# yeyupiaoling/VoiceprintRecognition-PaddlePaddle

Hardware: NVIDIA H100
Metric: utterances/sec ECAPA-TDNN Fbank80 3s embed extract (higher is better)
Workload: dtype bf16x3 (split-bf16 operands, fp32 accumulate; fp32-grade)

## Files before the change

voiceprintrecognition-paddlepaddle_b200/csrc/common.h:

```cpp
#pragma once
#include <cuda.h>
#include <cuda_bf16.h>
#include <cuda_runtime.h>
#include <stdint.h>
#include <stdlib.h>

#include <algorithm>
#include <string>
#include <utility>

#include "../../include/ppv_b200.h"

namespace ppv {

void set_error(const std::string& msg);
int fail(int code, const std::string& msg);

#define PPV_CUDA_OK(expr)                                                                             \
    do {                                                                                              \
        cudaError_t _e = (expr);                                                                      \
        if (_e != cudaSuccess)                                                                        \
            return ::ppv::fail(PPV_ECUDA, std::string(#expr) + ": " + cudaGetErrorString(_e));        \
    } while (0)
#define PPV_LAUNCH_OK(what)                                                                           \
// ... 134 lines not shown
    for (int bn = max_bn; bn > 64; bn /= 2)
        if (N % bn == 0) return bn;
    return 64;
}

int encode_planes_map(CUtensorMap* m, const Planes& t, int box_rows);
int encode_planes_map_ex(CUtensorMap* m, const Planes& t, int box_cols, int box_rows, int swizzle_bytes);

struct Res2Params {
    CUtensorMap mapA[2];
    CUtensorMap mapW;
    int a_col[2];
    int nsrc, dil;
    int l2_prefetch;
    int M, m_tiles;
    Epilogue epi;
};
int res2conv_build(Res2Params* rp, const GemmSource* srcs, int nsrc, const Planes& W, int M, int dil, const Epilogue& epi);
int res2conv_launch(const Res2Params& rp, int precision, int num_sms, cudaStream_t st);

struct Conv3x3Params {
    CUtensorMap mapX;
    CUtensorMap mapW;
    int x_col0;
    int B, H, W, Hp, Wp;
    int nph, npw, patches;
    Epilogue epi;
};
bool conv3x3_c32_supported(int Cin, int Cout, int H, int W);
int conv3x3_build(Conv3x3Params* cp, const Planes& x, int x_col0, const Planes& Wt, int B, int H, int W, int Hp, int Wp, const Epilogue& epi);
int conv3x3_launch(const Conv3x3Params& cp, int precision, int num_sms, cudaStream_t st);

constexpr int RES2CHAIN_MAX = 7;
struct Res2ChainParams {
    CUtensorMap mapX;
    CUtensorMap mapXt, mapY, mapYtail;
    CUtensorMap mapW[RES2CHAIN_MAX];
    const float* bias[RES2CHAIN_MAX];
    const float* bn_scale[RES2CHAIN_MAX];
    const float* bn_shift[RES2CHAIN_MAX];
    Planes x;
    Planes y;
    int nconv, width, B, T, P, Tp, dil, ntiles;
    int paired;
    unsigned long long* trace;
};
int res2chain_build(Res2ChainParams* cp, const Planes& x, const Planes& y, const Planes* W, const float* const* bias, const float* const* bn_scale,
                    const float* const* bn_shift, int nconv, int B, int T, int P, int Tp, int dil, bool paired);
int res2chain_launch(const Res2ChainParams& cp, int precision, int num_sms, cudaStream_t st);
bool res2chain_fits(int T, int P);
bool res2chain_pair_fits(int T, int P);
void res2chain_trace_dump(const Res2ChainParams& cp);

int pointwise_launch(const GemmSource* srcs, int nsrc, const Planes& W, int64_t M, int N, const Epilogue& ep, int num_sms, cudaStream_t st);
struct PwStep {
    GemmSource srcs[2];
    int nsrc = 0, N = 0;
    int64_t M = 0;
    Planes W;
    Epilogue ep;
};
inline int pointwise_launch(const PwStep& s, int num_sms, cudaStream_t st) { return pointwise_launch(s.srcs, s.nsrc, s.W, s.M, s.N, s.ep, num_sms, st); }
bool pointwise_step_build(PwStep* s, const GemmSource* srcs, int nsrc, const Planes& W, int N, int64_t M, const Epilogue& ep);

bool skinny_linear_supported(int M, int N, int K, const Epilogue& ep);
int skinny_linear_launch(const Planes& x, int x_col0, const Planes& W, int M, int N, int K, const Epilogue& ep, cudaStream_t st);

struct AspFusedParams {
    CUtensorMap mapW;
    CUtensorMap mapAtt;
    CUtensorMap mapX;
    Planes x;
    Planes gstat;
    const float* bn_scale;
    const float* bn_shift;
    Planes out;
    float* out_raw;
    int B, T, P, Tp, C, K;
    float eps;
    const int* nvalid;
};

int asp_fused_build(AspFusedParams* p, const Planes& W, const Planes& att, const Planes& x, const Planes& gstat, const float* bn_scale,
                    const float* bn_shift, const Planes& out, float* out_raw, int B, int T, int P, int Tp, int C, int K, float eps);
int asp_fused_launch(const AspFusedParams& p, int precision, int num_sms, cudaStream_t st);

int launch_pack_features(const float* feat, int B, int T, int F, const Planes& out, int P, int Tp, cudaStream_t st);
int launch_colstats(const Planes& x, int col0, int C, int B, int T, int P, int Tp, int mode, float eps, float* out_f32,
                    const Planes& out_pl, cudaStream_t st, float inv_count = 0.f, const int* nvalid = nullptr);
int launch_lengths_to_counts(const float* lengths, int B, int T, int* nvalid, cudaStream_t st);
int launch_se_scale_res(const Planes& z, const float* scale, const Planes& res, int rc0, const Planes& out, int oc0, int C,
                        int Tp, int64_t rows, int num_sms, cudaStream_t st, int relu = 0, float relu_max = 0.f);
int launch_asp_pool(const float* logits, int64_t lg_ld, const Planes& x, int C, int B, int T, int P, int Tp, float eps,
                    const float* bn_scale, const float* bn_shift, const Planes& out_pl, float* out_raw, cudaStream_t st);
int launch_planes_to_f32(const Planes& x, int col0, int C, int B, int T, int P, int Tp, float* out, cudaStream_t st);
int launch_f32_to_planes(const float* src, int64_t rows, int cols, const Planes& out, cudaStream_t st);

struct Fbank;
int fbank_create(const ppv_fbank_cfg* cfg, Fbank** out);
void fbank_destroy(Fbank* h);
int fbank_num_frames(const Fbank* h, int L);
int fbank_n_mels(const Fbank* h);
int fbank_run(Fbank* h, const float* wav, const float* lens_ratio, int B, int L, float* raw, float* out_f32,
              const Planes& out_pl, int P, int Tp, cudaStream_t st, const int* valid_frames = nullptr);

size_t audio_prep_workspace_bytes(int B, int max_new_len);
// ... 72 lines not shown
```

voiceprintrecognition-paddlepaddle_b200/csrc/ecapa.cu:

```cuda
#include <stdlib.h>
#include <string.h>

#include "common.h"
#include "model_common.h"

namespace ppv {

namespace {

struct ConvW : GemmWeights {
    float* bn_scale = nullptr;
    float* bn_shift = nullptr;
};

struct KSpec {
    int src;
    int col0, ncols, row_off;
    int w_cin0, w_cnt, w_tap;
};

enum Buf { B_FEAT, B_X0, B_H, B_Y, B_Z, B_CAT, B_MFA, B_ATT, B_GSTAT, B_POOL, B_SEM, B_SEH, B_COUNT };

struct Step {
    enum Kind { GEMM, SKINNY, RES2, RES2CHAIN, SE_SQUEEZE, SE_SCALE, ASP_GLOBAL, ASP_FUSED, POOL_STATS } kind;
    Planes sk_x, sk_w;
    int sk_col0 = 0, sk_M = 0, sk_N = 0, sk_K = 0;
    Epilogue sk_ep;
    GemmParams gp;
    AspFusedParams ap;
    Res2Params rp;
    Res2ChainParams cp;
    int blk = 0;
};

struct EcBuffers {
    Planes bufs[B_COUNT];
    float *se_mean = nullptr, *se_scale = nullptr, *fold_out = nullptr, *pooled_raw = nullptr, *raw_logmel = nullptr;
    int* nvalid = nullptr;
};

}

struct EcapaModel : Model {
    ppv_ecapa_cfg cfg;
    int C = 0, C3 = 0, width = 0, scale = 0, Fp = 0, P = 0, att = 0, se = 0;
    ConvW conv0, tdnn1[3], res2[3][8], tdnn2[3], se1[3], se2[3], mfa, fold, att1, att2, fc;
    float *aspbn_scale = nullptr, *aspbn_shift = nullptr;
    std::vector<Step> steps;
    EcBuffers buf;
    int Tp = 0;
    bool prof_on = false;
    std::vector<cudaEvent_t> prof_ev;
    std::vector<int> prof_kind;
    size_t prof_used = 0;
    int64_t launches_gemm = 0, launches_other = 0;

    explicit EcapaModel(const ppv_ecapa_cfg& c) : Model("ecapa", c.precision), cfg(c) {}
    ~EcapaModel() override {
        for (cudaEvent_t e : prof_ev) cudaEventDestroy(e);
    }
    int embd_dim() const override { return cfg.embd_dim; }
    size_t workspace_bytes(int B, int T) const override;
    int forward_ex(const float* feat, Fbank* fb, const float* wav, const float* lens_ratio, int B, int T, int L, float* emb, void* ws,
                   size_t ws_bytes, cudaStream_t st, const float* lengths);

  protected:
    bool prepare_weights(ArenaBuilder& ab) override;
    int build_plan(int B, int T, void* ws, size_t ws_bytes, cudaStream_t st) override;
    int run_steps(const float* feat, cudaStream_t st) override { return run(feat, nullptr, nullptr, nullptr, 0, nullptr, st); }
    int tap(const std::string& n, float* out, size_t out_elems, cudaStream_t st) override;
    int run(const float* feat, Fbank* fb, const float* wav, const float* lens_ratio, int L, const float* lengths, cudaStream_t st);
};

void ppv_ecapa_default_cfg_impl(ppv_ecapa_cfg* c) {
    c->input_size = 80;
    c->embd_dim = 192;
    const int ch[5] = {512, 512, 512, 512, 1536}, ks[5] = {5, 3, 3, 3, 1}, dl[5] = {1, 2, 3, 4, 1};
    for (int i = 0; i < 5; ++i) {
        c->channels[i] = ch[i];
        c->kernel_sizes[i] = ks[i];
        c->dilations[i] = dl[i];
    }
    c->attention_channels = 128;
    c->res2net_scale = 8;
// ... 175 lines not shown
    eb->bufs[B_H] = cv.planes(R, C);
    eb->bufs[B_Y] = cv.planes(R, C);
    eb->bufs[B_Z] = cv.planes(R, C);
    eb->bufs[B_CAT] = cv.planes(R, C3);
    eb->bufs[B_MFA] = cv.planes(R, C3);
    eb->bufs[B_ATT] = cv.planes(R, m->att);
    eb->bufs[B_GSTAT] = cv.planes(B, 2 * C3);
    eb->bufs[B_POOL] = cv.planes(B, 2 * C3);
    eb->bufs[B_SEM] = cv.planes(B, C);
    eb->bufs[B_SEH] = cv.planes(B, m->se);
    eb->se_mean = static_cast<float*>(cv.take(size_t(B) * C * 4));
    eb->se_scale = static_cast<float*>(cv.take(size_t(B) * C * 4));
    eb->fold_out = static_cast<float*>(cv.take(mc_align_up(B, 128) * m->att * 4));
    eb->pooled_raw = static_cast<float*>(cv.take(size_t(B) * 2 * C3 * 4));
    eb->raw_logmel = static_cast<float*>(cv.take(size_t(B) * T * m->cfg.input_size * 4));
    *emb_out = static_cast<float*>(cv.take(mc_align_up(B, 128) * m->cfg.embd_dim * 4));
    eb->nvalid = static_cast<int*>(cv.take(size_t(B) * sizeof(int)));
}

constexpr int ECAPA_MAX_BN = 128;

}

size_t EcapaModel::workspace_bytes(int B, int T) const {
    if (B <= 0 || T <= 0) return 0;
    WsCarver cv;
    EcBuffers eb;
    float* emb;
    carve(this, cv, B, T, &eb, &emb);
    return mc_align_up(cv.off, 256);
}

int EcapaModel::build_plan(int B, int T, void* ws, size_t ws_bytes, cudaStream_t st) {
    EcapaModel* const m = this;
    PPV_REQUIRE(T > m->P, "ecapa: too few frames for the reflect padding");
    const size_t need = workspace_bytes(B, T);
    PPV_REQUIRE(ws && ws_bytes >= need, "ecapa: workspace too small (see ppv_model_workspace_bytes)");
    PPV_REQUIRE((reinterpret_cast<uintptr_t>(ws) & 255) == 0, "ecapa: workspace must be 256-byte aligned");
    WsCarver cv;
    cv.base = static_cast<uint8_t*>(ws);
    carve(m, cv, B, T, &m->buf, &m->emb_out);
    m->Tp = T + 2 * m->P;
    PPV_CUDA_OK(cudaMemsetAsync(ws, 0, need, st));
    m->steps.clear();
    const int Tp = m->Tp, P = m->P, C = m->C, C3 = m->C3, w = m->width;
    const int64_t R = int64_t(B) * Tp;
    const char* r2env = getenv("PPV_RES2_GEMM");
    const bool use_res2_kernel = (w == 64) && !(r2env && r2env[0] == '1');
    const char* rcenv = getenv("PPV_RES2_CHAIN");
    const bool use_res2_chain = use_res2_kernel && m->scale == 8 && res2chain_fits(T, P) && !(rcenv && rcenv[0] == '0');
    const bool res2_paired = use_res2_chain && res2chain_pair_fits(T, P) && !(rcenv && strcmp(rcenv, "single") == 0);
    const char* skenv = getenv("PPV_SKINNY");
    const bool use_skinny = !(skenv && skenv[0] == '0');

    auto add_gemm = [&](const ConvW& cw, const std::vector<KSpec>& ks, const Planes* src_override, int override_col0, int M,
                        Epilogue ep) -> int {
        std::vector<GemmSource> srcs;
        for (const KSpec& s : ks) {
            GemmSource g;
            if (s.src < 0) {
                g.t = *src_override;
                g.col0 = override_col0 + s.col0;
            } else {
                g.t = m->buf.bufs[s.src];
                g.col0 = s.col0;
            }
            g.ncols = s.ncols;
            g.row_off = s.row_off;
            srcs.push_back(g);
        }
        ep.bias = cw.bias;
        if (ep.relu) {
            ep.bn_scale = cw.bn_scale;
            ep.bn_shift = cw.bn_shift;
        }
        if (use_skinny && M == B && srcs.size() == 1 && srcs[0].row_off == 0 && skinny_linear_supported(M, cw.N, srcs[0].ncols, ep) &&
            cw.Ktot == srcs[0].ncols) {
            Step sk;
            sk.kind = Step::SKINNY;
            sk.sk_x = srcs[0].t;
            sk.sk_col0 = srcs[0].col0;
            sk.sk_w = cw.W;
            sk.sk_M = M;
            sk.sk_N = cw.N;
            sk.sk_K = srcs[0].ncols;
            sk.sk_ep = ep;
            m->steps.push_back(sk);
            return PPV_OK;
        }
        Step stp;
        stp.kind = Step::GEMM;
        int rc = gemm_build(&stp.gp, srcs.data(), int(srcs.size()), cw.W, M, cw.N, ep, gemm_pick_bn(cw.N, ECAPA_MAX_BN));
        if (rc) return rc;
        m->steps.push_back(stp);
        return PPV_OK;
    };
    auto planes_out = [&](const Planes& p, int col0, bool halo) {
        Epilogue ep;
        ep.out_mode = OUT_PLANES;
        ep.out = p.base;
        ep.out_ld = p.ld;
        ep.out_plane_stride = p.plane_stride;
        ep.out_col0 = col0;
        ep.Tp = Tp;
        ep.P = P;
        ep.T = T;
        ep.halo = halo ? 1 : 0;
        ep.relu = 1;
        return ep;
    };
    int rc = add_gemm(m->conv0, spec_conv0(m), nullptr, 0, int(R), planes_out(m->buf.bufs[B_X0], 0, false));
    if (rc) return rc;
    for (int b = 1; b <= 3; ++b) {
        const Planes& X = (b == 1) ? m->buf.bufs[B_X0] : m->buf.bufs[B_CAT];
        const int xcol = (b == 1) ? 0 : (b - 2) * C;
        rc = add_gemm(m->tdnn1[b - 1], {{-1, 0, C, 0, 0, C, 0}}, &X, xcol, int(R), planes_out(m->buf.bufs[B_H], 0, !use_res2_chain));
        if (rc) return rc;
        if (use_res2_chain) {
            Planes Wj[RES2CHAIN_MAX];
            const float *bj[RES2CHAIN_MAX], *sj[RES2CHAIN_MAX], *hj[RES2CHAIN_MAX];
            for (int j = 1; j < m->scale; ++j) {
                const ConvW& cw = m->res2[b - 1][j];
                Wj[j - 1] = cw.W;
                bj[j - 1] = cw.bias;
                sj[j - 1] = cw.bn_scale;
                hj[j - 1] = cw.bn_shift;
            }
            Step stp;
            stp.kind = Step::RES2CHAIN;
            rc = res2chain_build(&stp.cp, m->buf.bufs[B_H], m->buf.bufs[B_Y], Wj, bj, sj, hj, m->scale - 1, B, T, P, Tp, m->cfg.dilations[b],
                                 res2_paired);
            if (rc) return rc;
            m->steps.push_back(stp);
        }
        for (int j = 1; j < m->scale && !use_res2_chain; ++j) {
            if (use_res2_kernel) {
                GemmSource srcs[2];
                srcs[0] = GemmSource{m->buf.bufs[B_H], j * w, w, 0};
                srcs[1] = GemmSource{m->buf.bufs[B_Y], (j - 1) * w, w, 0};
                Epilogue ep = planes_out(m->buf.bufs[B_Y], j * w, true);
                const ConvW& cw = m->res2[b - 1][j];
                ep.bias = cw.bias;
                ep.bn_scale = cw.bn_scale;
                ep.bn_shift = cw.bn_shift;
                Step stp;
                stp.kind = Step::RES2;
                rc = res2conv_build(&stp.rp, srcs, j >= 2 ? 2 : 1, cw.W, int(R), m->cfg.dilations[b], ep);
                if (rc) return rc;
                m->steps.push_back(stp);
            } else {
                rc = add_gemm(m->res2[b - 1][j], spec_res2(m, b, j), nullptr, 0, int(R), planes_out(m->buf.bufs[B_Y], j * w, true));
                if (rc) return rc;
            }
        }
        rc = add_gemm(m->tdnn2[b - 1], {{B_H, 0, w, 0, 0, w, 0}, {B_Y, w, C - w, 0, w, C - w, 0}}, nullptr, 0, int(R),
                      planes_out(m->buf.bufs[B_Z], 0, false));
        if (rc) return rc;
        Step s;
        s.blk = b;
        s.kind = Step::SE_SQUEEZE;
        m->steps.push_back(s);
        {
            Epilogue e1;
            e1.out_mode = OUT_PLANES;
            e1.out = m->buf.bufs[B_SEH].base;
            e1.out_ld = m->buf.bufs[B_SEH].ld;
            e1.out_plane_stride = m->buf.bufs[B_SEH].plane_stride;
            e1.relu = 1;
            rc = add_gemm(m->se1[b - 1], {{B_SEM, 0, C, 0, 0, 0, 0}}, nullptr, 0, B, e1);
            if (rc) return rc;
            Epilogue e2;
            e2.out_mode = OUT_F32;
            e2.out = m->buf.se_scale;
            e2.out_ld = C;
            e2.sigmoid_ = 1;
            rc = add_gemm(m->se2[b - 1], {{B_SEH, 0, m->se, 0, 0, 0, 0}}, nullptr, 0, B, e2);
            if (rc) return rc;
        }
        s.kind = Step::SE_SCALE;
        m->steps.push_back(s);
    }
    rc = add_gemm(m->mfa, {{B_CAT, 0, C3, 0, 0, C3, 0}}, nullptr, 0, int(R), planes_out(m->buf.bufs[B_MFA], 0, false));
    if (rc) return rc;
    const int pooling = m->cfg.pooling;
    if (pooling == PPV_POOL_TAP || pooling == PPV_POOL_TSP) {
        Step s;
        s.kind = Step::POOL_STATS;
        m->steps.push_back(s);
    } else {
        Step s;
        s.kind = Step::ASP_GLOBAL;
        m->steps.push_back(s);
    }
    if (pooling == PPV_POOL_ASP && m->cfg.global_context) {
        Epilogue ep;
        ep.out_mode = OUT_F32;
        ep.out = m->buf.fold_out;
        ep.out_ld = m->att;
        ConvW cw = m->fold;
        cw.bias = nullptr;
        rc = add_gemm(cw, {{B_GSTAT, 0, 2 * C3, 0, 0, 0, 0}}, nullptr, 0, B, ep);
        if (rc) return rc;
    }
    if (pooling == PPV_POOL_ASP || pooling == PPV_POOL_SAP) {
        {
            Epilogue ep = planes_out(m->buf.bufs[B_ATT], 0, false);
            if (pooling == PPV_POOL_ASP) {
// ... 38 lines not shown
    }
    rc = update_plan(B, T, ws, ws_bytes, st);
    if (!rc) rc = run(feat, fb, wav, lens_ratio, L, lengths, st);
    return rc ? rc : copy_embeddings(emb, st);
}

int ecapa_forward(Model* m, const float* feat, Fbank* fb, const float* wav, const float* lens_ratio, int B, int T, int L, float* emb, void* ws,
                  size_t ws_bytes, cudaStream_t st, const float* lengths) {
    return static_cast<EcapaModel*>(m)->forward_ex(feat, fb, wav, lens_ratio, B, T, L, emb, ws, ws_bytes, st, lengths);
}

int EcapaModel::run(const float* feat, Fbank* fb, const float* wav, const float* lens_ratio, int L, const float* lengths, cudaStream_t st) {
    EcapaModel* const m = this;
    const int B = m->plan_B, T = m->plan_T;
    const int Tp = m->Tp, P = m->P, C = m->C, C3 = m->C3;
    const int64_t R = int64_t(B) * Tp;
    int rc;
    auto prof_mark = [&](int kind, bool begin) {
        if (!m->prof_on) return;
        if (begin) {
            if (m->prof_used + 2 > m->prof_ev.size()) {
                cudaEvent_t a, b;
                cudaEventCreate(&a);
                cudaEventCreate(&b);
                m->prof_ev.push_back(a);
                m->prof_ev.push_back(b);
                m->prof_kind.push_back(kind);
            }
            m->prof_kind[m->prof_used / 2] = kind;
            cudaEventRecord(m->prof_ev[m->prof_used], st);
        } else {
            cudaEventRecord(m->prof_ev[m->prof_used + 1], st);
            m->prof_used += 2;
        }
    };
    const int* nv = nullptr;
    if (lengths) {
        PPV_REQUIRE(m->cfg.pooling == PPV_POOL_ASP, "ecapa_forward: lengths is implemented for ASP pooling (the other heads ignore it in the reference)");
        rc = launch_lengths_to_counts(lengths, B, T, m->buf.nvalid, st);
        if (rc) return rc;
        nv = m->buf.nvalid;
    }
    prof_mark(1, true);
    if (wav) {
        rc = fbank_run(fb, wav, lens_ratio, B, L, m->buf.raw_logmel, nullptr, m->buf.bufs[B_FEAT], P, Tp, st);
        m->launches_other += 3;
    } else {
        rc = launch_pack_features(feat, B, T, m->cfg.input_size, m->buf.bufs[B_FEAT], P, Tp, st);
        m->launches_other += 1;
    }
    prof_mark(1, false);
    if (rc) return rc;
    for (const Step& s : m->steps) {
        const bool tensor_step = (s.kind == Step::GEMM || s.kind == Step::ASP_FUSED || s.kind == Step::RES2 || s.kind == Step::RES2CHAIN);
        prof_mark(tensor_step ? 0 : 1, true);
        if (tensor_step) m->launches_gemm += 1; else m->launches_other += 1;
        switch (s.kind) {
            case Step::GEMM: rc = gemm_launch(s.gp, m->precision, m->num_sms, st); break;
            case Step::SKINNY: rc = skinny_linear_launch(s.sk_x, s.sk_col0, s.sk_w, s.sk_M, s.sk_N, s.sk_K, s.sk_ep, st); break;
            case Step::RES2: rc = res2conv_launch(s.rp, m->precision, m->num_sms, st); break;
            case Step::RES2CHAIN:
                rc = res2chain_launch(s.cp, m->precision, m->num_sms, st);
                if (s.cp.trace) {
                    static int dumps = 0;
                    if (++dumps == 10) res2chain_trace_dump(s.cp);
                }
                break;
            case Step::SE_SQUEEZE:
                rc = launch_colstats(m->buf.bufs[B_Z], 0, C, B, T, P, Tp, 0, 0.f, nullptr, m->buf.bufs[B_SEM], st, 0.f, nv);
                break;
            case Step::SE_SCALE: {
                const Planes& X = (s.blk == 1) ? m->buf.bufs[B_X0] : m->buf.bufs[B_CAT];
                const int xcol = (s.blk == 1) ? 0 : (s.blk - 2) * C;
                rc = launch_se_scale_res(m->buf.bufs[B_Z], m->buf.se_scale, X, xcol, m->buf.bufs[B_CAT], (s.blk - 1) * C, C, Tp, R, m->num_sms, st);
                break;
            }
            case Step::ASP_GLOBAL:
                rc = launch_colstats(m->buf.bufs[B_MFA], 0, C3, B, T, P, Tp, 1, 1e-12f, nullptr, m->buf.bufs[B_GSTAT], st, 0.f, nv);
                break;
            case Step::ASP_FUSED: {
                AspFusedParams ap = s.ap;
                ap.nvalid = nv;
                rc = asp_fused_launch(ap, m->precision, m->num_sms, st);
                break;
            }
            case Step::POOL_STATS:
                rc = launch_colstats(m->buf.bufs[B_MFA], 0, C3, B, T, P, Tp, m->cfg.pooling == PPV_POOL_TAP ? 0 : 3, 0.f, nullptr, m->buf.bufs[B_POOL], st);
                break;
        }
        prof_mark(0, false);
        if (rc) return rc;
    }
    return PPV_OK;
}

int ecapa_profile(Model* model, int enable) {
    EcapaModel* m = static_cast<EcapaModel*>(model);
    m->prof_on = enable != 0;
    m->prof_used = 0;
    m->launches_gemm = m->launches_other = 0;
    return PPV_OK;
}

int ecapa_profile_read(Model* model, double* gemm_ms, double* other_ms, int64_t* gemm_launches, int64_t* other_launches) {
    EcapaModel* m = static_cast<EcapaModel*>(model);
    PPV_REQUIRE(gemm_ms && other_ms && gemm_launches && other_launches, "ecapa_profile_read: null argument");
    double g = 0, o = 0;
    if (m->prof_used >= 2) PPV_CUDA_OK(cudaEventSynchronize(m->prof_ev[m->prof_used - 1]));
    for (size_t i = 0; i + 1 < m->prof_used; i += 2) {
        float ms = 0.f;
        PPV_CUDA_OK(cudaEventElapsedTime(&ms, m->prof_ev[i], m->prof_ev[i + 1]));
        (m->prof_kind[i / 2] == 0 ? g : o) += ms;
    }
    *gemm_ms = g;
    *other_ms = o;
    *gemm_launches = m->launches_gemm;
    *other_launches = m->launches_other;
    m->prof_used = 0;
    m->launches_gemm = m->launches_other = 0;
    return PPV_OK;
// ... 33 lines not shown
```

voiceprintrecognition-paddlepaddle_b200/csrc/ptx.cuh:

```cuda
#pragma once
#include <cuda.h>
#include <cuda_bf16.h>
#include <cuda_runtime.h>
#include <stdint.h>
#include <stdio.h>

namespace ppv {

__device__ __forceinline__ uint32_t smem_u32(const void* p) {
    return static_cast<uint32_t>(__cvta_generic_to_shared(p));
}

__device__ __forceinline__ bool elect_one() {
    uint32_t pred = 0;
    asm volatile(
        "{\n\t.reg .pred P;\n\t"
        "elect.sync _|P, 0xffffffff;\n\t"
        "selp.u32 %0, 1, 0, P;\n\t}\n"
        : "=r"(pred));
    return pred != 0;
}

__device__ __forceinline__ void mbar_init(uint32_t bar, uint32_t count) {
    asm volatile("mbarrier.init.shared::cta.b64 [%0], %1;" ::"r"(bar), "r"(count) : "memory");
}
__device__ __forceinline__ void fence_mbar_init() {
    asm volatile("fence.mbarrier_init.release.cluster;" ::: "memory");
}
__device__ __forceinline__ void mbar_arrive(uint32_t bar) {
    asm volatile("mbarrier.arrive.shared::cta.b64 _, [%0];" ::"r"(bar) : "memory");
}
__device__ __forceinline__ void mbar_arrive_expect_tx(uint32_t bar, uint32_t bytes) {
    asm volatile("mbarrier.arrive.expect_tx.shared::cta.b64 _, [%0], %1;" ::"r"(bar), "r"(bytes) : "memory");
}
__device__ __forceinline__ uint32_t mbar_try_wait(uint32_t bar, uint32_t parity) {
    uint32_t done;
    asm volatile(
        "{\n\t.reg .pred P;\n\t"
        "mbarrier.try_wait.parity.shared::cta.b64 P, [%1], %2;\n\t"
        "selp.u32 %0, 1, 0, P;\n\t}\n"
        : "=r"(done)
        : "r"(bar), "r"(parity)
        : "memory");
    return done;
}
__device__ __forceinline__ uint64_t global_timer_ns() {
    uint64_t t;
    asm volatile("mov.u64 %0, %%globaltimer;" : "=l"(t));
    return t;
}
__device__ __forceinline__ void mbar_wait(uint32_t bar, uint32_t parity) {
    if (mbar_try_wait(bar, parity)) return;
    const uint64_t t0 = global_timer_ns();
    uint32_t spins = 0;
    while (!mbar_try_wait(bar, parity)) {
        if ((++spins & 0x3ff) == 0 && global_timer_ns() - t0 > 4000000000ull) __trap();
    }
}

template <int N>
__device__ __forceinline__ void setmaxnreg_dec() { asm volatile("setmaxnreg.dec.sync.aligned.u32 %0;" ::"n"(N)); }
template <int N>
__device__ __forceinline__ void setmaxnreg_inc() { asm volatile("setmaxnreg.inc.sync.aligned.u32 %0;" ::"n"(N)); }

__device__ __forceinline__ void prefetch_tmap(const CUtensorMap* m) {
    asm volatile("prefetch.tensormap [%0];" ::"l"(reinterpret_cast<uint64_t>(m)) : "memory");
}
__device__ __forceinline__ void tma_load_3d(uint32_t smem_dst, const CUtensorMap* m, uint32_t bar, int c0, int c1,
                                            int c2) {
    asm volatile(
        "cp.async.bulk.tensor.3d.shared::cluster.global.mbarrier::complete_tx::bytes"
        " [%0], [%1, {%3, %4, %5}], [%2];"
        :
        : "r"(smem_dst), "l"(reinterpret_cast<uint64_t>(m)), "r"(bar), "r"(c0), "r"(c1), "r"(c2)
        : "memory");
}
__device__ __forceinline__ void tma_prefetch_l2_3d(const CUtensorMap* m, int c0, int c1, int c2) {
    asm volatile("cp.async.bulk.prefetch.tensor.3d.L2.global.tile [%0, {%1, %2, %3}];"
                 :
                 : "l"(reinterpret_cast<uint64_t>(m)), "r"(c0), "r"(c1), "r"(c2)
                 : "memory");
}
__device__ __forceinline__ void tma_store_3d(const CUtensorMap* m, uint32_t smem_src, int c0, int c1, int c2) {
    asm volatile("cp.async.bulk.tensor.3d.global.shared::cta.bulk_group [%0, {%2, %3, %4}], [%1];"
                 :
                 : "l"(reinterpret_cast<uint64_t>(m)), "r"(smem_src), "r"(c0), "r"(c1), "r"(c2)
                 : "memory");
}
__device__ __forceinline__ void bulk_commit_group() { asm volatile("cp.async.bulk.commit_group;" ::: "memory"); }
__device__ __forceinline__ void bulk_wait_read0() { asm volatile("cp.async.bulk.wait_group.read 0;" ::: "memory"); }
__device__ __forceinline__ void bulk_wait_all() { asm volatile("cp.async.bulk.wait_group 0;" ::: "memory"); }
__device__ __forceinline__ void fence_proxy_async_smem() { asm volatile("fence.proxy.async.shared::cta;" ::: "memory"); }
__device__ __forceinline__ void bulk_load_1d(uint32_t smem_dst, const void* gsrc, uint32_t bytes, uint32_t bar) {
    asm volatile(
        "cp.async.bulk.shared::cluster.global.mbarrier::complete_tx::bytes [%0], [%1], %2, [%3];"
        :
        : "r"(smem_dst), "l"(reinterpret_cast<uint64_t>(gsrc)), "r"(bytes), "r"(bar)
        : "memory");
}

__device__ __forceinline__ void wgmma_fence() { asm volatile("wgmma.fence.sync.aligned;" ::: "memory"); }
__device__ __forceinline__ void wgmma_commit() { asm volatile("wgmma.commit_group.sync.aligned;" ::: "memory"); }
template <int N>
__device__ __forceinline__ void wgmma_wait() { asm volatile("wgmma.wait_group.sync.aligned %0;" ::"n"(N) : "memory"); }
template <int R>
__device__ __forceinline__ void wgmma_fence_acc(float (&d)[R]) {
#pragma unroll
    for (int i = 0; i < R; ++i) asm volatile("" : "+f"(d[i])::"memory");
}
__device__ __forceinline__ void wgmma_m64n32k16(float (&d)[16], uint64_t desc_a, uint64_t desc_b, uint32_t scale_d) {
    asm volatile(
        "{\n\t.reg .pred p;\n\t"
// ... 113 lines not shown
```

Measured before the change: 45310.

## Fuse TDNN2 conv, SE squeeze/excite and residual scale into one cluster kernel

Adds a 4-CTA cluster kernel that runs the tdnn2 pointwise GEMM with bias, ReLU and BN, then computes the SE time means, the hidden and scale layers, and applies the sigmoid scale plus residual add. CTAs in a cluster exchange partial means and hidden activations through distributed shared memory. This replaces the separate GEMM, colstats, SE and scale launches per block, removing the write and reread of the Z intermediate and several launches. The cost is that each cluster processes whole utterances (T up to 320), so parallelism is limited to the number of clusters that fit, and the per-utterance phases run serially.

```diff
diff --git a/voiceprintrecognition-paddlepaddle_b200/csrc/common.h b/voiceprintrecognition-paddlepaddle_b200/csrc/common.h
--- a/voiceprintrecognition-paddlepaddle_b200/csrc/common.h
+++ b/voiceprintrecognition-paddlepaddle_b200/csrc/common.h
@@ -210,6 +210,25 @@
 bool res2chain_pair_fits(int T, int P);
 void res2chain_trace_dump(const Res2ChainParams& cp);
 
+struct SeTailParams {
+    CUtensorMap mapA[2];
+    CUtensorMap mapW;
+    CUtensorMap mapX;
+    const float *bias, *bn_scale, *bn_shift;
+    Planes w1, w2;
+    const float *b1, *b2;
+    Planes x, out;
+    int x_col0, out_col0;
+    int h_cols, B, T, P, Tp;
+    const int* nvalid;
+    unsigned long long* trace;
+};
+bool se_tail_supported(int C, int S, int T);
+int se_tail_build(SeTailParams* p, const Planes& h, const Planes& y, int h_cols, const Planes& W, const float* bias, const float* bn_scale,
+                  const float* bn_shift, const Planes& w1, const float* b1, const Planes& w2, const float* b2, const Planes& x, int x_col0,
+                  const Planes& out, int out_col0, int B, int T, int P, int Tp);
+int se_tail_launch(const SeTailParams& p, int precision, cudaStream_t st);
+
 int pointwise_launch(const GemmSource* srcs, int nsrc, const Planes& W, int64_t M, int N, const Epilogue& ep, int num_sms, cudaStream_t st);
 struct PwStep {
     GemmSource srcs[2];
diff --git a/voiceprintrecognition-paddlepaddle_b200/csrc/ecapa.cu b/voiceprintrecognition-paddlepaddle_b200/csrc/ecapa.cu
--- a/voiceprintrecognition-paddlepaddle_b200/csrc/ecapa.cu
+++ b/voiceprintrecognition-paddlepaddle_b200/csrc/ecapa.cu
@@ -22,7 +22,7 @@
 enum Buf { B_FEAT, B_X0, B_H, B_Y, B_Z, B_CAT, B_MFA, B_ATT, B_GSTAT, B_POOL, B_SEM, B_SEH, B_COUNT };
 
 struct Step {
-    enum Kind { GEMM, SKINNY, RES2, RES2CHAIN, SE_SQUEEZE, SE_SCALE, ASP_GLOBAL, ASP_FUSED, POOL_STATS } kind;
+    enum Kind { GEMM, SKINNY, RES2, RES2CHAIN, SE_TAIL, SE_SQUEEZE, SE_SCALE, ASP_GLOBAL, ASP_FUSED, POOL_STATS } kind;
     Planes sk_x, sk_w;
     int sk_col0 = 0, sk_M = 0, sk_N = 0, sk_K = 0;
     Epilogue sk_ep;
@@ -30,6 +30,7 @@
     AspFusedParams ap;
     Res2Params rp;
     Res2ChainParams cp;
+    SeTailParams tp;
     int blk = 0;
 };
 
@@ -311,6 +312,8 @@
     const bool res2_paired = use_res2_chain && res2chain_pair_fits(T, P) && !(rcenv && strcmp(rcenv, "single") == 0);
     const char* skenv = getenv("PPV_SKINNY");
     const bool use_skinny = !(skenv && skenv[0] == '0');
+    const char* stenv = getenv("PPV_SE_TAIL");
+    const bool use_se_tail = se_tail_supported(C, m->se, T) && !(stenv && stenv[0] == '0');
 
     auto add_gemm = [&](const ConvW& cw, const std::vector<KSpec>& ks, const Planes* src_override, int override_col0, int M,
                         Epilogue ep) -> int {
@@ -412,6 +415,16 @@
                 if (rc) return rc;
             }
         }
+        if (use_se_tail) {
+            Step stp;
+            stp.kind = Step::SE_TAIL;
+            const ConvW &t2 = m->tdnn2[b - 1], &s1 = m->se1[b - 1], &s2 = m->se2[b - 1];
+            rc = se_tail_build(&stp.tp, m->buf.bufs[B_H], m->buf.bufs[B_Y], w, t2.W, t2.bias, t2.bn_scale, t2.bn_shift, s1.W, s1.bias, s2.W, s2.bias, X,
+                               xcol, m->buf.bufs[B_CAT], (b - 1) * C, B, T, P, Tp);
+            if (rc) return rc;
+            m->steps.push_back(stp);
+            continue;
+        }
         rc = add_gemm(m->tdnn2[b - 1], {{B_H, 0, w, 0, 0, w, 0}, {B_Y, w, C - w, 0, w, C - w, 0}}, nullptr, 0, int(R),
                       planes_out(m->buf.bufs[B_Z], 0, false));
         if (rc) return rc;
@@ -556,7 +569,8 @@
     prof_mark(1, false);
     if (rc) return rc;
     for (const Step& s : m->steps) {
-        const bool tensor_step = (s.kind == Step::GEMM || s.kind == Step::ASP_FUSED || s.kind == Step::RES2 || s.kind == Step::RES2CHAIN);
+        const bool tensor_step = (s.kind == Step::GEMM || s.kind == Step::ASP_FUSED || s.kind == Step::RES2 || s.kind == Step::RES2CHAIN ||
+                                  s.kind == Step::SE_TAIL);
         prof_mark(tensor_step ? 0 : 1, true);
         if (tensor_step) m->launches_gemm += 1; else m->launches_other += 1;
         switch (s.kind) {
@@ -570,6 +584,12 @@
                     if (++dumps == 10) res2chain_trace_dump(s.cp);
                 }
                 break;
+            case Step::SE_TAIL: {
+                SeTailParams tp = s.tp;
+                tp.nvalid = nv;
+                rc = se_tail_launch(tp, m->precision, st);
+                break;
+            }
             case Step::SE_SQUEEZE:
                 rc = launch_colstats(m->buf.bufs[B_Z], 0, C, B, T, P, Tp, 0, 0.f, nullptr, m->buf.bufs[B_SEM], st, 0.f, nv);
                 break;
diff --git a/voiceprintrecognition-paddlepaddle_b200/csrc/ptx.cuh b/voiceprintrecognition-paddlepaddle_b200/csrc/ptx.cuh
--- a/voiceprintrecognition-paddlepaddle_b200/csrc/ptx.cuh
+++ b/voiceprintrecognition-paddlepaddle_b200/csrc/ptx.cuh
@@ -58,6 +58,55 @@
     }
 }
 
+__device__ __forceinline__ uint32_t cluster_ctarank() {
+    uint32_t r;
+    asm volatile("mov.u32 %0, %%cluster_ctarank;" : "=r"(r));
+    return r;
+}
+__device__ __forceinline__ uint32_t cluster_id_x() {
+    uint32_t r;
+    asm volatile("mov.u32 %0, %%clusterid.x;" : "=r"(r));
+    return r;
+}
+__device__ __forceinline__ uint32_t cluster_count_x() {
+    uint32_t r;
+    asm volatile("mov.u32 %0, %%nclusterid.x;" : "=r"(r));
+    return r;
+}
+__device__ __forceinline__ void cluster_sync() {
+    asm volatile("barrier.cluster.arrive.release.aligned;\n\tbarrier.cluster.wait.acquire.aligned;" ::: "memory");
+}
+__device__ __forceinline__ uint32_t mapa_shared(uint32_t addr, uint32_t rank) {
+    uint32_t r;
+    asm volatile("mapa.shared::cluster.u32 %0, %1, %2;" : "=r"(r) : "r"(addr), "r"(rank));
+    return r;
+}
+__device__ __forceinline__ void st_shared_cluster_f32(uint32_t addr, float v) {
+    asm volatile("st.shared::cluster.f32 [%0], %1;" ::"r"(addr), "f"(v) : "memory");
+}
+__device__ __forceinline__ void mbar_arrive_cluster(uint32_t cluster_bar) {
+    asm volatile("mbarrier.arrive.release.cluster.shared::cluster.b64 _, [%0];" ::"r"(cluster_bar) : "memory");
+}
+__device__ __forceinline__ uint32_t mbar_try_wait_cluster(uint32_t bar, uint32_t parity) {
+    uint32_t done;
+    asm volatile(
+        "{\n\t.reg .pred P;\n\t"
+        "mbarrier.try_wait.parity.acquire.cluster.shared::cta.b64 P, [%1], %2;\n\t"
+        "selp.u32 %0, 1, 0, P;\n\t}\n"
+        : "=r"(done)
+        : "r"(bar), "r"(parity)
+        : "memory");
+    return done;
+}
+__device__ __forceinline__ void mbar_wait_cluster(uint32_t bar, uint32_t parity) {
+    if (mbar_try_wait_cluster(bar, parity)) return;
+    const uint64_t t0 = global_timer_ns();
+    uint32_t spins = 0;
+    while (!mbar_try_wait_cluster(bar, parity)) {
+        if ((++spins & 0x3ff) == 0 && global_timer_ns() - t0 > 4000000000ull) __trap();
+    }
+}
+
 template <int N>
 __device__ __forceinline__ void setmaxnreg_dec() { asm volatile("setmaxnreg.dec.sync.aligned.u32 %0;" ::"n"(N)); }
 template <int N>
diff --git a/voiceprintrecognition-paddlepaddle_b200/csrc/se_tail.cu b/voiceprintrecognition-paddlepaddle_b200/csrc/se_tail.cu
--- /dev/null
+++ b/voiceprintrecognition-paddlepaddle_b200/csrc/se_tail.cu
@@ -0,0 +1,450 @@
+#include <stdio.h>
+#include <stdlib.h>
+#include <string.h>
+
+#include "common.h"
+#include "gemm_epilogue.cuh"
+#include "ptx.cuh"
+
+namespace ppv {
+
+namespace {
+
+constexpr int ST_CLUSTER = 4;
+constexpr int ST_C = 512;
+constexpr int ST_S = 128;
+constexpr int ST_COLS = ST_C / ST_CLUSTER;
+constexpr int ST_HID = ST_S / ST_CLUSTER;
+constexpr int ST_MB = 5;
+constexpr int ST_ROWS = 64 * ST_MB;
+constexpr int ST_BK = 32;
+constexpr int ST_NK = ST_C / ST_BK;
+constexpr int ST_ABOX = ST_ROWS / 2;
+constexpr int ST_THREADS = 384;
+constexpr int ST_RING_BYTES = 172032;
+constexpr int ST_XBOX_BYTES = ST_ABOX * 64 * 2;
+constexpr int ST_X_BYTES = 8 * ST_XBOX_BYTES;
+static_assert(ST_X_BYTES <= ST_RING_BYTES, "the residual slab must fit in the ring");
+constexpr int ST_SCRATCH_FLOATS = 3 * ST_COLS + 4 * ST_COLS + ST_C + ST_S + ST_COLS;
+constexpr int ST_BAR_BYTES = 256;
+
+template <int NSPLIT>
+struct SeTailCfg {
+    static constexpr int NP = (NSPLIT == 3) ? 2 : 1;
+    static constexpr int A_PLANE = ST_ROWS * ST_BK * 2;
+    static constexpr int W_PLANE = ST_COLS * ST_BK * 2;
+    static constexpr int STAGE_BYTES = NP * (A_PLANE + W_PLANE);
+    static constexpr int STAGES = ST_RING_BYTES / STAGE_BYTES > 8 ? 8 : ST_RING_BYTES / STAGE_BYTES;
+    static constexpr int SMEM_BYTES = 1024 + ST_RING_BYTES + ST_SCRATCH_FLOATS * 4 + ST_BAR_BYTES;
+    static_assert(STAGES >= 2, "need at least a double buffer");
+    static_assert(SMEM_BYTES <= 232448, "shared memory");
+};
+
+template <int NSPLIT>
+__global__ void __launch_bounds__(ST_THREADS, 1) se_tail_kernel(const __grid_constant__ SeTailParams p) {
+    using Cfg = SeTailCfg<NSPLIT>;
+    constexpr int STAGES = Cfg::STAGES;
+    extern __shared__ uint8_t smem_raw[];
+    const uint32_t base = (smem_u32(smem_raw) + 1023u) & ~1023u;
+    float* const s_bias = reinterpret_cast<float*>(smem_raw + (base - smem_u32(smem_raw)) + ST_RING_BYTES);
+    float* const s_bnsc = s_bias + ST_COLS;
+    float* const s_bnsh = s_bnsc + ST_COLS;
+    float* const s_part = s_bnsh + ST_COLS;
+    float* const s_mall = s_part + 4 * ST_COLS;
+    float* const s_hall = s_mall + ST_C;
+    float* const s_scale = s_hall + ST_S;
+    const uint32_t bar_base = base + ST_RING_BYTES + ST_SCRATCH_FLOATS * 4;
+    auto full_bar = [&](int s) { return bar_base + 8u * s; };
+    auto empty_bar = [&](int s) { return bar_base + 8u * (8 + s); };
+    const uint32_t mean_bar = bar_base + 8u * 16;
+    const uint32_t hid_bar = bar_base + 8u * 17;
+    const uint32_t x_full = bar_base + 8u * 18;
+    const uint32_t x_empty = bar_base + 8u * 19;
+    const uint8_t* const ring = smem_raw + (base - smem_u32(smem_raw));
+
+    const int warp = threadIdx.x >> 5, lane = threadIdx.x & 31;
+    const uint32_t rank = cluster_ctarank();
+    const int n0 = int(rank) * ST_COLS;
+    if (threadIdx.x == 0) {
+        prefetch_tmap(&p.mapA[0]);
+        prefetch_tmap(&p.mapA[1]);
+        prefetch_tmap(&p.mapW);
+        prefetch_tmap(&p.mapX);
+    }
+    if (warp == 1 && lane == 0) {
+        for (int s = 0; s < STAGES; ++s) {
+            mbar_init(full_bar(s), 1);
+            mbar_init(empty_bar(s), 2);
+        }
+        mbar_init(mean_bar, ST_COLS * ST_CLUSTER);
+        mbar_init(hid_bar, ST_HID * ST_CLUSTER);
+        mbar_init(x_full, 1);
+        mbar_init(x_empty, 256);
+        fence_mbar_init();
+    }
+    if (threadIdx.x < ST_COLS) {
+        s_bias[threadIdx.x] = p.bias[n0 + threadIdx.x];
+        s_bnsc[threadIdx.x] = p.bn_scale[n0 + threadIdx.x];
+        s_bnsh[threadIdx.x] = p.bn_shift[n0 + threadIdx.x];
+    }
+    cluster_sync();
+    griddep_launch_dependents();
+    griddep_wait();
+
+    const int cid = int(cluster_id_x()), ncl = int(cluster_count_x());
+    const bool trace_cta = p.trace != nullptr && cid == 0 && rank == 0;
+    auto stamp = [&](bool on, int u, int e) {
+        if (on && u < 8) p.trace[8 * u + e] = clock64();
+    };
+    if (trace_cta && threadIdx.x == 0) p.trace[64] = clock64();
+
+    if (warp < 4) {
+        setmaxnreg_dec<40>();
+        if (warp == 0 && lane == 0) {
+            int stage = 0;
+            uint32_t phase = 0;
+            for (int b = cid, u = 0; b < p.B; b += ncl, ++u) {
+                const int row0 = b * p.Tp + p.P;
+#pragma unroll
+                for (int pl = 0; pl < 2; ++pl)
+#pragma unroll
+                    for (int i = 0; i < 4; ++i) tma_prefetch_l2_3d(&p.mapX, p.x_col0 + n0 + 64 * (i & 1), row0 + ST_ABOX * (i >> 1), pl);
+                for (int s = 0; s < ST_NK; ++s) {
+                    mbar_wait(empty_bar(stage), phase ^ 1u);
+                    stamp(trace_cta && s == 0, u, 7);
+                    const uint32_t sa = base + stage * Cfg::STAGE_BYTES;
+                    const uint32_t sw = sa + Cfg::NP * Cfg::A_PLANE;
+                    const uint32_t fb = full_bar(stage);
+                    mbar_arrive_expect_tx(fb, Cfg::STAGE_BYTES);
+                    const int kc = s * ST_BK;
+                    const CUtensorMap* ma = kc < p.h_cols ? &p.mapA[0] : &p.mapA[1];
+#pragma unroll
+                    for (int pl = 0; pl < Cfg::NP; ++pl) {
+                        tma_load_3d(sa + pl * Cfg::A_PLANE, ma, fb, kc, row0, pl);
+                        tma_load_3d(sa + pl * Cfg::A_PLANE + ST_ABOX * ST_BK * 2, ma, fb, kc, row0 + ST_ABOX, pl);
+                        tma_load_3d(sw + pl * Cfg::W_PLANE, &p.mapW, fb, kc, n0, pl);
+                    }
+                    if (++stage == STAGES) {
+                        stage = 0;
+                        phase ^= 1u;
+                    }
+                }
+                for (int i = 0, st2 = stage; i < STAGES; ++i, st2 = st2 + 1 == STAGES ? 0 : st2 + 1)
+                    mbar_wait(empty_bar(st2), (st2 >= stage ? phase : phase ^ 1u) ^ 1u);
+                mbar_arrive_expect_tx(x_full, ST_X_BYTES);
+#pragma unroll
+                for (int i = 0; i < 8; ++i)
+                    tma_load_3d(base + i * ST_XBOX_BYTES, &p.mapX, x_full, p.x_col0 + n0 + 64 * ((i >> 1) & 1), row0 + ST_ABOX * (i & 1), i >> 2);
+                mbar_wait(x_empty, uint32_t(u & 1));
+            }
+        }
+        return;
+    }
+
+    setmaxnreg_inc<232>();
+    const int g = (warp - 4) >> 2;
+    const int mt = threadIdx.x - 128;
+    const int t = threadIdx.x & 127;
+    const int w = t >> 5, q = lane & 3;
+    int stage = 0;
+    uint32_t phase = 0, uphase = 0;
+    float acc[ST_MB][32];
+#pragma unroll
+    for (int mb = 0; mb < ST_MB; ++mb)
+#pragma unroll
+        for (int i = 0; i < 32; ++i) acc[mb][i] = 0.f;
+    int u = 0;
+    for (int b = cid; b < p.B; b += ncl, uphase ^= 1u, ++u) {
+        const bool tr = trace_cta && mt == 0;
+        int prev = -1;
+#pragma unroll
+        for (int mb = 0; mb < ST_MB; ++mb) wgmma_fence_acc(acc[mb]);
+        for (int s = 0; s < ST_NK; ++s) {
+            mbar_wait(full_bar(stage), phase);
+            stamp(tr && s == 0, u, 0);
+            const uint32_t sa = base + stage * Cfg::STAGE_BYTES;
+            const uint32_t sw = sa + Cfg::NP * Cfg::A_PLANE + g * 64 * ST_BK * 2;
+            const uint64_t b_hi = make_sw64_kmajor_desc(sw);
+            const uint64_t b_lo = make_sw64_kmajor_desc(sw + Cfg::W_PLANE);
+            wgmma_fence();
+#pragma unroll
+            for (int mb = 0; mb < ST_MB; ++mb) {
+                const uint64_t a_hi = make_sw64_kmajor_desc(sa + mb * 64 * ST_BK * 2);
+#pragma unroll
+                for (int k = 0; k < ST_BK / 16; ++k) wgmma_bf16<64>(acc[mb], a_hi + 2 * k, b_hi + 2 * k, (s > 0 || k > 0) ? 1u : 0u);
+                if (NSPLIT == 3) {
+                    const uint64_t a_lo = make_sw64_kmajor_desc(sa + Cfg::A_PLANE + mb * 64 * ST_BK * 2);
+#pragma unroll
+                    for (int k = 0; k < ST_BK / 16; ++k) wgmma_bf16<64>(acc[mb], a_lo + 2 * k, b_hi + 2 * k, 1u);
+#pragma unroll
+                    for (int k = 0; k < ST_BK / 16; ++k) wgmma_bf16<64>(acc[mb], a_hi + 2 * k, b_lo + 2 * k, 1u);
+                }
+            }
+            wgmma_commit();
+            wgmma_wait<1>();
+            if (prev >= 0 && t == 0) mbar_arrive(empty_bar(prev));
+            prev = stage;
+            if (++stage == STAGES) {
+                stage = 0;
+                phase ^= 1u;
+            }
+        }
+        wgmma_wait<0>();
+#pragma unroll
+        for (int mb = 0; mb < ST_MB; ++mb) wgmma_fence_acc(acc[mb]);
+        if (t == 0) mbar_arrive(empty_bar(prev));
+        stamp(tr, u, 1);
+
+        const int T = p.T;
+        const int n = p.nvalid ? max(1, min(T, p.nvalid[b])) : T;
+        float csum[16];
+#pragma unroll
+        for (int j = 0; j < 16; ++j) csum[j] = 0.f;
+#pragma unroll
+        for (int mb = 0; mb < ST_MB; ++mb) {
+            const int ta = 64 * mb + 16 * w + (lane >> 2);
+            const bool va = ta < n, vb = ta + 8 < n;
+#pragma unroll
+            for (int i = 0; i < 8; ++i)
+#pragma unroll
+                for (int e = 0; e < 2; ++e) {
+                    const int c = 64 * g + 8 * i + 2 * q + e;
+                    const float bb = s_bias[c], sc = s_bnsc[c], sh = s_bnsh[c];
+                    float& za = acc[mb][4 * i + e];
+                    float& zb = acc[mb][4 * i + 2 + e];
+                    za = fmaf(fmaxf(za + bb, 0.f), sc, sh);
+                    zb = fmaf(fmaxf(zb + bb, 0.f), sc, sh);
+                    csum[2 * i + e] += va ? za : 0.f;
+                    csum[2 * i + e] += vb ? zb : 0.f;
+                }
+        }
+#pragma unroll
+        for (int j = 0; j < 16; ++j) {
+            float v = csum[j];
+            v += __shfl_xor_sync(0xffffffffu, v, 4);
+            v += __shfl_xor_sync(0xffffffffu, v, 8);
+            v += __shfl_xor_sync(0xffffffffu, v, 16);
+            csum[j] = v;
+        }
+        if ((lane >> 2) == 0) {
+#pragma unroll
+            for (int i = 0; i < 8; ++i)
+#pragma unroll
+                for (int e = 0; e < 2; ++e) s_part[w * ST_COLS + 64 * g + 8 * i + 2 * q + e] = csum[2 * i + e];
+        }
+        named_bar_sync(1, 256);
+        stamp(tr, u, 2);
+        if (mt < ST_COLS) {
+            const float m = ((s_part[mt] + s_part[ST_COLS + mt]) + (s_part[2 * ST_COLS + mt] + s_part[3 * ST_COLS + mt])) / float(n);
+            const uint32_t dst = smem_u32(s_mall + n0 + mt);
+#pragma unroll
+            for (uint32_t r = 0; r < ST_CLUSTER; ++r) {
+                st_shared_cluster_f32(mapa_shared(dst, r), m);
+                mbar_arrive_cluster(mapa_shared(mean_bar, r));
+            }
+        }
+        mbar_wait_cluster(mean_bar, uphase);
+        stamp(tr, u, 3);
+        {
+            const int j = ST_HID * int(rank) + (mt >> 3), part = mt & 7;
+            const int64_t off = int64_t(j) * p.w1.ld + 64 * part;
+            const float* mv = s_mall + 64 * part;
+            float a = 0.f;
+#pragma unroll 2
+            for (int k8 = 0; k8 < 8; ++k8) {
+                const uint4 h = __ldg(reinterpret_cast<const uint4*>(p.w1.hi() + off + 8 * k8));
+                const uint4 l = __ldg(reinterpret_cast<const uint4*>(p.w1.lo() + off + 8 * k8));
+                const uint32_t hw[4] = {h.x, h.y, h.z, h.w}, lw[4] = {l.x, l.y, l.z, l.w};
+#pragma unroll
+                for (int e = 0; e < 4; ++e) {
+                    const float2 wh = unpack_bf16x2(hw[e]), wl = unpack_bf16x2(lw[e]);
+                    a = fmaf(wh.x + wl.x, mv[8 * k8 + 2 * e], a);
+                    a = fmaf(wh.y + wl.y, mv[8 * k8 + 2 * e + 1], a);
+                }
+            }
+            a += __shfl_xor_sync(0xffffffffu, a, 1);
+            a += __shfl_xor_sync(0xffffffffu, a, 2);
+            a += __shfl_xor_sync(0xffffffffu, a, 4);
+            if (part == 0) {
+                const float hv = fmaxf(a + __ldg(p.b1 + j), 0.f);
+                const uint32_t dst = smem_u32(s_hall + j);
+#pragma unroll
+                for (uint32_t r = 0; r < ST_CLUSTER; ++r) {
+                    st_shared_cluster_f32(mapa_shared(dst, r), hv);
+                    mbar_arrive_cluster(mapa_shared(hid_bar, r));
+                }
+            }
+        }
+        mbar_wait_cluster(hid_bar, uphase);
+        stamp(tr, u, 4);
+        {
+            const int c = mt >> 1, half = mt & 1;
+            const int64_t off = int64_t(n0 + c) * p.w2.ld + 64 * half;
+            const float* hv = s_hall + 64 * half;
+            float a = 0.f;
+#pragma unroll 2
+            for (int k8 = 0; k8 < 8; ++k8) {
+                const uint4 h = __ldg(reinterpret_cast<const uint4*>(p.w2.hi() + off + 8 * k8));
+                const uint4 l = __ldg(reinterpret_cast<const uint4*>(p.w2.lo() + off + 8 * k8));
+                const uint32_t hw[4] = {h.x, h.y, h.z, h.w}, lw[4] = {l.x, l.y, l.z, l.w};
+#pragma unroll
+                for (int e = 0; e < 4; ++e) {
+                    const float2 wh = unpack_bf16x2(hw[e]), wl = unpack_bf16x2(lw[e]);
+                    a = fmaf(wh.x + wl.x, hv[8 * k8 + 2 * e], a);
+                    a = fmaf(wh.y + wl.y, hv[8 * k8 + 2 * e + 1], a);
+                }
+            }
+            a += __shfl_xor_sync(0xffffffffu, a, 1);
+            if (half == 0) s_scale[c] = 1.f / (1.f + expf(-(a + __ldg(p.b2 + n0 + c))));
+        }
+        named_bar_sync(1, 256);
+        stamp(tr, u, 5);
+        const int64_t row0 = int64_t(b) * p.Tp + p.P;
+        mbar_wait(x_full, uphase);
+#pragma unroll
+        for (int mb = 0; mb < ST_MB; ++mb) {
+            const int ta = 64 * mb + 16 * w + (lane >> 2);
+#pragma unroll
+            for (int hh = 0; hh < 2; ++hh) {
+                float za[8], zb[8];
+#pragma unroll
+                for (int i = 0; i < 4; ++i) {
+                    za[2 * i] = acc[mb][4 * (4 * hh + i)], za[2 * i + 1] = acc[mb][4 * (4 * hh + i) + 1];
+                    zb[2 * i] = acc[mb][4 * (4 * hh + i) + 2], zb[2 * i + 1] = acc[mb][4 * (4 * hh + i) + 3];
+                }
+                quad_transpose_pairs(za, zb, q);
+                const int c = 64 * g + 32 * hh + 8 * q;
+                float sv[8];
+#pragma unroll
+                for (int k = 0; k < 8; ++k) sv[k] = s_scale[c + k];
+                auto store_row = [&](int tr, const float(&z)[8]) {
+                    if (tr >= T) return;
+                    const int rr = tr % ST_ABOX;
+                    const int xoff = (2 * g + tr / ST_ABOX) * ST_XBOX_BYTES + rr * 128 + (((4 * hh + q) ^ (rr & 7)) << 4);
+                    const uint4 xh = *reinterpret_cast<const uint4*>(ring + xoff);
+                    const uint4 xl = *reinterpret_cast<const uint4*>(ring + 4 * ST_XBOX_BYTES + xoff);
+                    const uint32_t hw[4] = {xh.x, xh.y, xh.z, xh.w}, lw[4] = {xl.x, xl.y, xl.z, xl.w};
+                    uint32_t oh[4], ol[4];
+#pragma unroll
+                    for (int e = 0; e < 4; ++e) {
+                        const float2 a = unpack_bf16x2(hw[e]), bl = unpack_bf16x2(lw[e]);
+                        const float y0 = fmaf(sv[2 * e], z[2 * e], a.x + bl.x), y1 = fmaf(sv[2 * e + 1], z[2 * e + 1], a.y + bl.y);
+                        split_pack_bf16x2(y0, y1, oh[e], ol[e]);
+                    }
+                    const int64_t oo = (row0 + tr) * p.out.ld + p.out_col0 + n0 + c;
+                    *reinterpret_cast<uint4*>(p.out.hi() + oo) = make_uint4(oh[0], oh[1], oh[2], oh[3]);
+                    *reinterpret_cast<uint4*>(p.out.lo() + oo) = make_uint4(ol[0], ol[1], ol[2], ol[3]);
+                };
+                store_row(ta, za);
+                store_row(ta + 8, zb);
+            }
+        }
+        mbar_arrive(x_empty);
+        stamp(tr, u, 6);
+    }
+}
+
+}
+
+bool se_tail_supported(int C, int S, int T) { return C == ST_C && S == ST_S && T >= 1 && T <= ST_ROWS; }
+
+int se_tail_build(SeTailParams* p, const Planes& h, const Planes& y, int h_cols, const Planes& W, const float* bias, const float* bn_scale,
+                  const float* bn_shift, const Planes& w1, const float* b1, const Planes& w2, const float* b2, const Planes& x, int x_col0,
+                  const Planes& out, int out_col0, int B, int T, int P, int Tp) {
+    PPV_REQUIRE(se_tail_supported(W.ld, w2.ld, T), "se_tail: C = 512, S = 128 and T <= 320 required");
+    PPV_REQUIRE(h_cols > 0 && h_cols % ST_BK == 0 && h_cols < ST_C && h.ld >= h_cols && y.ld >= ST_C, "se_tail: source columns");
+    PPV_REQUIRE(W.rows >= ST_C && w1.ld == ST_C && w1.rows >= ST_S && w2.rows >= ST_C, "se_tail: weight shapes");
+    PPV_REQUIRE(x.ld % 8 == 0 && out.ld % 8 == 0 && x_col0 % 8 == 0 && out_col0 % 8 == 0 && x.plane_stride % 8 == 0 &&
+                    out.plane_stride % 8 == 0 && (reinterpret_cast<uintptr_t>(x.base) & 15) == 0 &&
+                    (reinterpret_cast<uintptr_t>(out.base) & 15) == 0 && x_col0 + ST_C <= x.ld && out_col0 + ST_C <= out.ld,
+                "se_tail: residual / output must be 16-byte aligned");
+    PPV_REQUIRE(bias && bn_scale && bn_shift && b1 && b2, "se_tail: missing bias / BatchNorm vectors");
+    memset(p, 0, sizeof(*p));
+    int rc = encode_planes_map_ex(&p->mapA[0], h, ST_BK, ST_ABOX, 64);
+    if (!rc) rc = encode_planes_map_ex(&p->mapA[1], y, ST_BK, ST_ABOX, 64);
+    if (!rc) rc = encode_planes_map_ex(&p->mapW, W, ST_BK, ST_COLS, 64);
+    if (!rc) rc = encode_planes_map_ex(&p->mapX, x, 64, ST_ABOX, 128);
+    if (rc) return rc;
+    p->bias = bias;
+    p->bn_scale = bn_scale;
+    p->bn_shift = bn_shift;
+    p->w1 = w1;
+    p->w2 = w2;
+    p->b1 = b1;
+    p->b2 = b2;
+    p->x = x;
+    p->out = out;
+    p->x_col0 = x_col0;
+    p->out_col0 = out_col0;
+    p->h_cols = h_cols;
+    p->B = B;
+    p->T = T;
+    p->P = P;
+    p->Tp = Tp;
+    if (getenv("PPV_SE_TAIL_TRACE")) {
+        static unsigned long long* buf = nullptr;
+        if (!buf) {
+            PPV_CUDA_OK(cudaMalloc(reinterpret_cast<void**>(&buf), 72 * sizeof(unsigned long long)));
+            PPV_CUDA_OK(cudaMemset(buf, 0, 72 * sizeof(unsigned long long)));
+        }
+        p->trace = buf;
+    }
+    return PPV_OK;
+}
+
+template <int NSPLIT>
+static int se_tail_launch_t(const SeTailParams& p, cudaStream_t st) {
+    using Cfg = SeTailCfg<NSPLIT>;
+    PPV_ONCE_PER_DEVICE(PPV_CUDA_OK(cudaFuncSetAttribute(se_tail_kernel<NSPLIT>, cudaFuncAttributeMaxDynamicSharedMemorySize, Cfg::SMEM_BYTES)));
+    cudaLaunchConfig_t cfg = {};
+    cfg.gridDim = dim3(ST_CLUSTER);
+    cfg.blockDim = dim3(ST_THREADS);
+    cfg.dynamicSmemBytes = Cfg::SMEM_BYTES;
+    cfg.stream = st;
+    cudaLaunchAttribute attr[2];
+    attr[0].id = cudaLaunchAttributeClusterDimension;
+    attr[0].val.clusterDim.x = ST_CLUSTER;
+    attr[0].val.clusterDim.y = 1;
+    attr[0].val.clusterDim.z = 1;
+    attr[1].id = cudaLaunchAttributeProgrammaticStreamSerialization;
+    attr[1].val.programmaticStreamSerializationAllowed = pdl_enabled() ? 1 : 0;
+    cfg.attrs = attr;
+    cfg.numAttrs = 2;
+    static int max_clusters[64] = {0};
+    int dev = 0;
+    PPV_CUDA_OK(cudaGetDevice(&dev));
+    int& mc = max_clusters[dev & 63];
+    if (mc == 0) {
+        PPV_CUDA_OK(cudaOccupancyMaxActiveClusters(&mc, se_tail_kernel<NSPLIT>, &cfg));
+        PPV_REQUIRE(mc > 0, "se_tail: no 4-CTA cluster fits on this device");
+    }
+    cfg.gridDim = dim3(ST_CLUSTER * std::min(p.B, mc));
+    PPV_PDL_OK(cudaLaunchKernelEx(&cfg, se_tail_kernel<NSPLIT>, p), "se_tail_kernel");
+    if (p.trace) {
+        static int launches = 0;
+        if (++launches == 10) {
+            unsigned long long h[72];
+            PPV_CUDA_OK(cudaDeviceSynchronize());
+            PPV_CUDA_OK(cudaMemcpy(h, p.trace, sizeof(h), cudaMemcpyDeviceToHost));
+            printf("se_tail trace: %d clusters of %d CTAs, B = %d, T = %d (cycles from kernel start)\n", mc, ST_CLUSTER, p.B, p.T);
+            printf("se_tail trace   slot_free  first_k    kloop_end  sums       means      hidden     scales     stores\n");
+            for (int u = 0; u < 8; ++u) {
+                if (!h[8 * u + 1]) continue;
+                const long long e[8] = {(long long)(h[8 * u + 7] - h[64]), (long long)(h[8 * u] - h[64]), (long long)(h[8 * u + 1] - h[64]),
+                                        (long long)(h[8 * u + 2] - h[64]), (long long)(h[8 * u + 3] - h[64]), (long long)(h[8 * u + 4] - h[64]),
+                                        (long long)(h[8 * u + 5] - h[64]), (long long)(h[8 * u + 6] - h[64])};
+                printf("se_tail trace u%d", u);
+                for (int i = 0; i < 8; ++i) printf(" %10lld", e[i]);
+                printf("\n");
+            }
+            fflush(stdout);
+        }
+    }
+    return PPV_OK;
+}
+
+int se_tail_launch(const SeTailParams& p, int precision, cudaStream_t st) {
+    return precision == PPV_PREC_BF16X3 ? se_tail_launch_t<3>(p, st) : se_tail_launch_t<1>(p, st);
+}
+
+}
```

Result: faster. 46150, median of 6 (+1.9%).
